# SinOncology/BreakID

Measured on NVIDIA B200. Metric: read_pairs_per_sec_classified_clustered_refined, higher is better.
Workload: dtype u32/i64 integer + f64 (AHC distances)

## Files before the change

### breakid_b200/csrc/bkid_api.cuh

```cuda
#pragma once

#define GRID1(n, t) (unsigned)div_up((long long)(n), (t))

enum CounterSlot {
  CS_G = 0,
  CS_SD_OUT = 16,
  CS_SDF = 20,
  CS_SORT = 28,
  CS_TOTAL = 32,
  CS_HASH_ERR = 40,
  CS_MAXSPAN = 44,
  CS_FATAL = 46,
  CS_ROOTS = 48,
  CS_MISSING = 50,
  CS_DECODE = 52,
  CS_NC = 64,
  CS_XBAD = 65,
  CS_RG_TICKET = 66,
  CS_SORT_HEAP = 67
};

struct Scratch {
  DBuf keys, keys_alt, vals, vals_alt, hist, scan_tmp, a32, b32, c32, d32, e32;
  int ensure(long long n, cudaStream_t st)
// ... 197 lines not shown
  cudaStream_t st = c->st;
  if (n == 0) { CU(c, cudaMemsetAsync(seg_out, 0, (size_t)(nseg + 1) * 4, st)); *n_out = 0; return 0; }
  TRY(c, c->sc.ensure(n, st));
  uint32_t *cnt = c->sc.a32.as<uint32_t>(), *off = c->sc.b32.as<uint32_t>();
  unsigned long long *tot = (unsigned long long *)(c->counters.as<unsigned>() + CS_TOTAL);
  BK_LAUNCH(k4_mask_count, GRID1(n, 256), 256, 0, st, cur, curb, seg, n, X, Y, distance, cnt);
  bk::exclusive_scan<uint32_t, uint32_t>(cnt, off, n, c->sc.scan_tmp.as<unsigned long long>(), tot, st);
  unsigned long long h = 0;
  CU(c, cudaMemcpyAsync(&h, tot, 8, cudaMemcpyDeviceToHost, st));
  CU(c, cudaStreamSynchronize(st));
  BK_LAUNCH(k4_mask_write, GRID1(n, 256), 256, 0, st, cur, curb, n, cnt, off, cur_out, curb_out);
  BK_LAUNCH(k4_new_offsets, GRID1(nseg + 1, 256), 256, 0, st, seg, nseg, off, n, h, seg_out);
  *n_out = (long long)h;
  return 0;
}

static int compact_pass(bkid_ctx *c, const uint32_t *cur, const uint32_t *curb, const uint32_t *seg, long long n, int nseg, const uint32_t *keep,
                        uint32_t *cur_out, uint32_t *curb_out, uint32_t *seg_out, uint32_t *off_keep , long long *n_out)
{
  cudaStream_t st = c->st;
  if (n == 0) { CU(c, cudaMemsetAsync(seg_out, 0, (size_t)(nseg + 1) * 4, st)); *n_out = 0; return 0; }
  unsigned long long *tot = (unsigned long long *)(c->counters.as<unsigned>() + CS_TOTAL);
  bk::exclusive_scan<uint32_t, uint32_t>(keep, off_keep, n, c->sc.scan_tmp.as<unsigned long long>(), tot, st);
  unsigned long long h = 0;
  CU(c, cudaMemcpyAsync(&h, tot, 8, cudaMemcpyDeviceToHost, st));
  CU(c, cudaStreamSynchronize(st));
  BK_LAUNCH(compact_write, GRID1(n, 256), 256, 0, st, cur, curb, keep, off_keep, n, cur_out, curb_out);
  BK_LAUNCH(k4_new_offsets, GRID1(nseg + 1, 256), 256, 0, st, seg, nseg, off_keep, n, h, seg_out);
  *n_out = (long long)h;
  return 0;
}

static int remove_isolated_all(bkid_ctx *c, const uint32_t *cur0, const uint32_t *curb0, const uint32_t *seg0, long long n0, int nseg,
                               const uint32_t *X, const uint32_t *Y, double w)
{
  cudaStream_t st = c->st;
  long long distance = (long long)w;
  size_t m = (size_t)std::max<long long>(n0, 1) * 4 + 64, sb = (size_t)(nseg + 2) * 4;
  TRY(c, c->cur1.ensure(m, 0, st)); TRY(c, c->curb1.ensure(m, 0, st)); TRY(c, c->seg1.ensure(sb, 0, st));
  DBuf &ca = c->sc.c32, &cb = c->sc.d32;
  TRY(c, c->sc.ensure(n0 + 8, st));
  TRY(c, c->tmpG.ensure(3 * sb + m * 2, 0, st));
  uint32_t *segA = c->tmpG.as<uint32_t>(), *segB = segA + (nseg + 2);
  uint32_t *curA = ca.as<uint32_t>(), *curbA = cb.as<uint32_t>();
  uint32_t *work_cur = c->tmpG.as<uint32_t>() + 3 * (nseg + 2);
  uint32_t *work_curb = work_cur + std::max<long long>(n0, 1) + 8;
  if (n0 > 0) {
    CU(c, cudaMemcpyAsync(work_cur, cur0, (size_t)n0 * 4, cudaMemcpyDeviceToDevice, st));
    CU(c, cudaMemcpyAsync(work_curb, curb0, (size_t)n0 * 4, cudaMemcpyDeviceToDevice, st));
  }
  TRY(c, sort_current_by(c, work_cur, n0, X, seg0, nseg));
  long long na = 0, nb2 = 0;
  TRY(c, mask_pass(c, work_cur, work_curb, seg0, n0, nseg, X, Y, distance, curA, curbA, segA, &na));
  TRY(c, sort_current_by(c, curA, na, Y, segA, nseg));
  TRY(c, mask_pass(c, curA, curbA, segA, na, nseg, X, Y, distance, c->cur1.as<uint32_t>(), c->curb1.as<uint32_t>(), segB, &nb2));
  TRY(c, sort_current_by(c, c->cur1.as<uint32_t>(), nb2, X, segB, nseg));
  CU(c, cudaMemcpyAsync(c->seg1.p, segB, (size_t)(nseg + 1) * 4, cudaMemcpyDeviceToDevice, st));
  c->n1 = nb2;
  return 0;
}

static int cluster_ahc(bkid_ctx *c, const uint32_t *cur, const uint32_t *curb, const uint32_t *seg, long long n, int nseg, const uint32_t *X, const uint32_t *Y, double thr_d)
{
  cudaStream_t st = c->st;
  c->n2 = 0;
  c->roots_per_bucket.assign(nseg, 0);
  if (n == 0) return 0;
  long long thr = (long long)thr_d;
  SubTimer T_(st);
  TRY(c, c->sc.ensure(n + 8, st));
  DBuf &LX = c->tmpA, &LY = c->tmpB;
  TRY(c, LX.ensure((size_t)n * 4 + 16, 0, st)); TRY(c, LY.ensure((size_t)n * 4 + 16, 0, st));
  BK_LAUNCH(gather_u32, GRID1(n, 256), 256, 0, st, X, cur, n, LX.as<uint32_t>());
  BK_LAUNCH(gather_u32, GRID1(n, 256), 256, 0, st, Y, cur, n, LY.as<uint32_t>());
  uint64_t *key = c->sc.keys.as<uint64_t>();
  uint32_t *val = c->sc.vals.as<uint32_t>();
  uint32_t *head = c->sc.a32.as<uint32_t>(), *hex = c->sc.b32.as<uint32_t>();
  unsigned long long *stmp = c->sc.scan_tmp.as<unsigned long long>();
  unsigned long long *tot = (unsigned long long *)(c->counters.as<unsigned>() + CS_TOTAL);
  int bbits = 1; while ((1ll << bbits) < nseg + 1) ++bbits;
  BK_LAUNCH(ahc_key_bx, GRID1(n, 256), 256, 0, st, curb, LX.as<uint32_t>(), n, key, val);
  bk::radix_sort_pairs(key, val, n, 0, 32 + bbits, c->sc.rt(), st);
  BK_LAUNCH(ahc_gap_heads, GRID1(n, 256), 256, 0, st, key, n, thr, head);
  bk::exclusive_scan<uint32_t, uint32_t>(head, hex, n, stmp, tot, st);
  unsigned long long npiece = 0;
  CU(c, cudaMemcpyAsync(&npiece, tot, 8, cudaMemcpyDeviceToHost, st)); CU(c, cudaStreamSynchronize(st));
  int pbits = 1; while ((1ull << pbits) < npiece + 1) ++pbits;
  BK_LAUNCH(ahc_key_group, GRID1(n, 256), 256, 0, st, head, hex, val, LY.as<uint32_t>(), n, key);
  bk::radix_sort_pairs(key, val, n, 0, 32 + pbits, c->sc.rt(), st);
  BK_LAUNCH(ahc_gap_heads, GRID1(n, 256), 256, 0, st, key, n, thr, head);
  bk::exclusive_scan<uint32_t, uint32_t>(head, hex, n, stmp, tot, st);
  unsigned long long ncomp64 = 0;
  CU(c, cudaMemcpyAsync(&ncomp64, tot, 8, cudaMemcpyDeviceToHost, st)); CU(c, cudaStreamSynchronize(st));
  uint32_t ncomp = (uint32_t)ncomp64;
  int cbits = 1; while ((1ull << cbits) < ncomp64 + 1) ++cbits;
  BK_LAUNCH(ahc_key_group, GRID1(n, 256), 256, 0, st, head, hex, val, (const uint32_t *)nullptr, n, key);
  bk::radix_sort_pairs(key, val, n, 0, 32 + cbits, c->sc.rt(), st);
  BK_LAUNCH(ahc_comp_heads, GRID1(n, 256), 256, 0, st, key, n, head);
  T_.mark("ahc: component sorts");
  DBuf &T = c->tmpC;
  size_t nc1 = (size_t)ncomp + 2;
  size_t bytes = nc1 * (4 + 4 + 4 + 8 + 8 + 8 + 8 + 4 + 8 + 8 + 4 + 8 + 4 + 4) + (size_t)n * (4 + 4 + 4) + (size_t)(nseg + 2) * (4 + 4 + 4 + 4) + 4096;
  TRY(c, T.ensure(bytes, 0, st));
  CU(c, cudaMemsetAsync(T.p, 0, bytes, st));
  char *bp = (char *)T.p;
  auto take = [&](size_t b) { char *r = bp; bp += (b + 15) & ~(size_t)15; return r; };
  uint32_t *comp_off = (uint32_t *)take(nc1 * 4), *comp_bucket = (uint32_t *)take(nc1 * 4);
  int32_t *hi_oc = (int32_t *)take(nc1 * 4);
  unsigned long long *pts_sz = (unsigned long long *)take(nc1 * 8), *row_sz = (unsigned long long *)take(nc1 * 8);
  unsigned long long *pts_off = (unsigned long long *)take(nc1 * 8), *row_off = (unsigned long long *)take(nc1 * 8);
  uint32_t *comp_nnodes = (uint32_t *)take(nc1 * 4);
  unsigned long long *comp_pts_used = (unsigned long long *)take(nc1 * 8), *comp_row_used = (unsigned long long *)take(nc1 * 8);
  int32_t *comp_head_j = (int32_t *)take(nc1 * 4);
  double *comp_head_d = (double *)take(nc1 * 8);
  int32_t *comp_flag = (int32_t *)take(nc1 * 4);
  uint32_t *comp_cursor = (uint32_t *)take(nc1 * 4);
  uint32_t *comp_of_point = (uint32_t *)take((size_t)n * 4);
  uint32_t *comp_leaf = (uint32_t *)take((size_t)n * 4);
  int32_t *lo_oc = (int32_t *)take((size_t)n * 4);
  uint32_t *bucket_comp_off = (uint32_t *)take((size_t)(nseg + 2) * 4);
  int32_t *bucket_flag = (int32_t *)take((size_t)(nseg + 2) * 4);
  unsigned *merges_pb = (unsigned *)take((size_t)(nseg + 2) * 4);
  uint32_t *bucket_first_root = (uint32_t *)take((size_t)(nseg + 2) * 4);
  BK_LAUNCH(ahc_comp_fill, GRID1(n, 256), 256, 0, st, key, head, val, n, curb, comp_off, comp_bucket, comp_of_point);
  CU(c, cudaMemcpyAsync(comp_leaf, val, (size_t)n * 4, cudaMemcpyDeviceToDevice, st));
  { uint32_t nn = (uint32_t)n; CU(c, cudaMemcpyAsync(comp_off + ncomp, &nn, 4, cudaMemcpyHostToDevice, st)); CU(c, cudaStreamSynchronize(st)); }
  BK_LAUNCH(ahc_comp_static, GRID1(ncomp, 128), 128, 0, st, comp_off, comp_leaf, comp_bucket, comp_of_point, seg, ncomp, lo_oc, hi_oc, pts_sz, row_sz);
  unsigned long long *tot2 = tot + 1;
  bk::exclusive_scan<unsigned long long, unsigned long long>(pts_sz, pts_off, ncomp, stmp, tot, st);
  bk::exclusive_scan<unsigned long long, unsigned long long>(row_sz, row_off, ncomp, stmp, tot2, st);
  unsigned long long pool[2] = {0, 0};
  std::vector<uint32_t> seg_h((size_t)nseg + 1);
  CU(c, cudaMemcpyAsync(seg_h.data(), seg, (size_t)(nseg + 1) * 4, cudaMemcpyDeviceToHost, st));
  CU(c, cudaMemcpyAsync(pool, tot, 16, cudaMemcpyDeviceToHost, st)); CU(c, cudaStreamSynchronize(st));
  bool have_large = false;
  const uint32_t RG_LO = 512u;
  for (int b = 0; b < nseg; ++b) have_large |= seg_h[b + 1] - seg_h[b] >= RG_LO;
  if ((pool[0] * 4 + pool[1] * 12) > (100ull << 30)) return fail(c, BKID_ERR_NOMEM, "AHC component too large for the row pools");
  BK_LAUNCH(ahc_bucket_comp_off, GRID1(nseg + 1, 128), 128, 0, st, comp_bucket, ncomp, (uint32_t)nseg, bucket_comp_off);
  DBuf &NB = c->tmpD;
  size_t nn2 = (size_t)2 * n + 2;
  size_t nbytes = nn2 * (1 + 4 + 8 + 8 + 4 + 4 + 8 + 4 + 4 + 4) + (size_t)n * (8 + 4) + pool[0] * 4 + pool[1] * 12 + 8192;
  TRY(c, NB.ensure(nbytes, 0, st));
  bp = (char *)NB.p;
  AhcView v;
  memset(&v, 0, sizeof v);
  v.seg_off = seg; v.X = LX.as<uint32_t>(); v.Y = LY.as<uint32_t>();
  v.comp_off = comp_off; v.comp_leaf = comp_leaf; v.comp_bucket = comp_bucket; v.lo_oc = lo_oc; v.hi_oc = hi_oc;
  v.pts_off = pts_off; v.row_off = row_off;
  v.node_best_d = (double *)take(nn2 * 8);
  v.node_pts = (unsigned long long *)take(nn2 * 8); v.node_row = (unsigned long long *)take(nn2 * 8);
  v.row_d = (double *)take(pool[1] * 8 + 8);
  v.ev_d = (double *)take((size_t)n * 8 + 8);
  v.node_npts = (uint32_t *)take(nn2 * 4); v.node_rowlen = (uint32_t *)take(nn2 * 4);
  v.node_best_t = (int32_t *)take(nn2 * 4); v.node_grank = (int32_t *)take(nn2 * 4);
  v.node_ma = (int32_t *)take(nn2 * 4); v.node_mb = (int32_t *)take(nn2 * 4);
  v.pts_pool = (uint32_t *)take(pool[0] * 4 + 8); v.row_t = (int32_t *)take(pool[1] * 4 + 8);
  v.ev_first = (int32_t *)take((size_t)n * 4 + 8);
  v.node_root = (uint8_t *)take(nn2);
  v.comp_nnodes = comp_nnodes; v.comp_pts_used = comp_pts_used; v.comp_row_used = comp_row_used;
  v.comp_head_j = comp_head_j; v.comp_head_d = comp_head_d; v.comp_flag = comp_flag; v.comp_cursor = comp_cursor;
  v.thr = (double)thr;
  T_.mark("ahc: tables+alloc");
  BK_LAUNCH(ahc_components, GRID1(ncomp, 4), 128, 0, st, v, ncomp);
  T_.mark("ahc: components kernel");
  BK_LAUNCH(ahc_bucket_flags, GRID1(ncomp, 128), 128, 0, st, comp_flag, comp_bucket, ncomp, bucket_flag);
  T_.mark("ahc: bucket flags");
  if (T_.on) {
    std::vector<int32_t> hf(ncomp); std::vector<uint32_t> hoff(ncomp + 1), hnn(ncomp);
    cudaMemcpyAsync(hf.data(), comp_flag, (size_t)ncomp * 4, cudaMemcpyDeviceToHost, st);
    cudaMemcpyAsync(hoff.data(), comp_off, (size_t)(ncomp + 1) * 4, cudaMemcpyDeviceToHost, st);
    cudaMemcpyAsync(hnn.data(), comp_nnodes, (size_t)ncomp * 4, cudaMemcpyDeviceToHost, st);
    cudaStreamSynchronize(st);
    long nf = 0, maxc = 0, merges = 0, fl_pts = 0;
    for (uint32_t i = 0; i < ncomp; ++i) { uint32_t cs = hoff[i + 1] - hoff[i]; nf += hf[i] != 0; if (hf[i]) fl_pts += cs; maxc = std::max<long>(maxc, cs); merges += hnn[i] - cs; }
    fprintf(stderr, "[bkid-timing] ncomp %u flagged %ld (points %ld) max comp %ld merges %ld points %lld buckets %d\n", ncomp, nf, fl_pts, maxc, merges, n, nseg);
  }
  BK_LAUNCH(ahc_replay_rank, (unsigned)nseg, RK_THREADS, 49 * 512, st, v, bucket_comp_off, (uint32_t)nseg, bucket_flag, 0u, RG_LO);
  T_.mark("ahc: replay rank form");
  BK_LAUNCH(ahc_replay_smem, (unsigned)nseg, 32, 49 * 900, st, v, bucket_comp_off, (uint32_t)nseg, bucket_flag, 0u, 900u);
  BK_LAUNCH(ahc_replay_smem, (unsigned)nseg, 32, 49 * 4096, st, v, bucket_comp_off, (uint32_t)nseg, bucket_flag, 900u, 4096u);
  T_.mark("ahc: replay smem (flagged)");
  if (have_large) {
    DBuf &RG = c->tmpF;
    size_t nn = (size_t)n + 8;
    TRY(c, RG.ensure(nn * (8 + 4 + 4 + 4 + 4 + 4 + 4 + 1) + (size_t)(nseg + 2) * 4 + 256, 0, st));
    char *q = (char *)RG.p;
    RankGlobal g;
    g.pm = (double *)q; q += nn * 8;
    g.slot_comp = (uint32_t *)q; q += nn * 4;
    g.first = (int32_t *)q; q += nn * 4;
    g.rank = (uint32_t *)q; q += nn * 4;
    g.order = (uint32_t *)q; q += nn * 4;
    g.is_head = (uint32_t *)q; q += nn * 4;
    uint32_t *head_excl = (uint32_t *)q; q += nn * 4;
    uint32_t *bucket_events = (uint32_t *)q; q += (size_t)(nseg + 2) * 4;
    g.tie = (uint8_t *)q;
    uint32_t *head_pos = c->sc.e32.as<uint32_t>();
    CU(c, cudaMemsetAsync(bucket_events, 0, (size_t)(nseg + 2) * 4, st));
    CU(c, cudaMemsetAsync(g.is_head, 0, nn * 4, st));
    BK_LAUNCH(ahc_rg_bucket_events, GRID1(ncomp, 128), 128, 0, st, v, ncomp, bucket_events);
    BK_LAUNCH(ahc_rg_prepare, GRID1(ncomp, 128), 128, 0, st, v, g, ncomp, bucket_flag, RG_LO);
    {
      uint64_t *rk = c->sc.keys.as<uint64_t>();
      uint32_t *rv = c->sc.vals.as<uint32_t>();
      BK_LAUNCH(ahc_rg_sortkeys, GRID1(n, 256), 256, 0, st, v, g, curb, n, bucket_flag, RG_LO, rk, rv);
      bk::radix_sort_pairs(rk, rv, n, 0, 64, c->sc.rt(), st);
      BK_LAUNCH(ahc_rg_bucketkeys, GRID1(n, 256), 256, 0, st, curb, rv, n, rk);
      bk::radix_sort_pairs(rk, rv, n, 0, bbits, c->sc.rt(), st);
// ... 1579 lines not shown
```

### breakid_b200/csrc/bkid_cluster.cuh

```cuda
#pragma once

struct AhcView {
  const uint32_t *seg_off;
  const uint32_t *X, *Y;
  const uint32_t *comp_off;
  const uint32_t *comp_leaf;
  const uint32_t *comp_bucket;
  const int32_t *lo_oc;
  const int32_t *hi_oc;
  const unsigned long long *pts_off, *row_off;
  uint8_t *node_root;
  uint32_t *node_npts;
  unsigned long long *node_pts;
  unsigned long long *node_row;
  uint32_t *node_rowlen;
  int32_t *node_best_t;
  double *node_best_d;
  int32_t *node_grank;
  int32_t *node_ma, *node_mb;
  uint32_t *pts_pool;
  int32_t *row_t;
  double *row_d;
  uint32_t *comp_nnodes;
  unsigned long long *comp_pts_used, *comp_row_used;
// ... 568 lines not shown
  uint32_t b = point_bucket[e];
  if (bucket_flag[b] || v.seg_off[b + 1] - v.seg_off[b] < n_lo) return;
  if (!(g.pm[e] < 1.0e300)) return;
  uint32_t comp = g.slot_comp[e], lbase = v.comp_off[comp], c = v.comp_off[comp + 1] - lbase;
  v.node_grank[2 * lbase + c + ((uint32_t)e - lbase)] = (int32_t)g.rank[e];
}

__global__ void __launch_bounds__(32) ahc_bucket_exact(AhcView v, const uint32_t *__restrict__ bucket_comp_off, uint32_t nb, const int32_t *__restrict__ bucket_flag, uint32_t n_lo)
{
  uint32_t b = blockIdx.x;
  if (b >= nb || !bucket_flag[b]) return;
  if (v.seg_off[b + 1] - v.seg_off[b] < n_lo) return;
  const unsigned lane = threadIdx.x & 31;
  uint32_t c0 = bucket_comp_off[b], c1 = bucket_comp_off[b + 1];
  uint32_t nleaf = v.seg_off[b + 1] - v.seg_off[b];
  for (uint32_t comp = c0; comp < c1; ++comp) {
    CompCtx cc = make_cc(v, comp);
    ahc_comp_init(v, cc);
    for (uint32_t j = 1; j < cc.c; ++j) ahc_find_best<true>(v, cc, j);
    ahc_comp_head(v, cc);
  }
  int32_t g = 0;
  while (true) {
    double bd = 1.7976931348623157e308; int32_t bg = -1; uint32_t bc = 0xffffffffu;
    for (uint32_t comp = c0 + lane; comp < c1; comp += 32) {
      int32_t hj = v.comp_head_j[comp];
      if (hj < 0) continue;
      uint32_t lbase = v.comp_off[comp], c = v.comp_off[comp + 1] - lbase;
      double d = v.comp_head_d[comp];
      int32_t gi = (uint32_t)hj < c ? (int32_t)(v.comp_leaf[lbase + hj] - v.seg_off[b]) : (int32_t)nleaf + v.node_grank[2 * lbase + hj];
      if (bg < 0 || d < bd || (d == bd && gi > bg)) { bd = d; bg = gi; bc = comp; }
    }
    for (int o = 16; o; o >>= 1) {
      double od = __shfl_xor_sync(0xffffffffu, bd, o);
      int32_t og = __shfl_xor_sync(0xffffffffu, bg, o);
      uint32_t oc = __shfl_xor_sync(0xffffffffu, bc, o);
      if (og >= 0 && (bg < 0 || od < bd || (od == bd && og > bg))) { bd = od; bg = og; bc = oc; }
    }
    if (bg < 0 || !(bd <= v.thr)) break;
    CompCtx cc = make_cc(v, bc);
    ahc_merge<true>(v, cc, g);
    ++g;
  }
}

__global__ void ahc_key_bx(const uint32_t *__restrict__ bucket_of, const uint32_t *__restrict__ X, long long np, uint64_t *__restrict__ key, uint32_t *__restrict__ val)
{
  long long p = (long long)blockIdx.x * blockDim.x + threadIdx.x;
  if (p < np) { key[p] = ((uint64_t)bucket_of[p] << 32) | X[p]; val[p] = (uint32_t)p; }
}
__global__ void ahc_gap_heads(const uint64_t *__restrict__ key, long long np, long long thr, uint32_t *__restrict__ head)
{
  long long p = (long long)blockIdx.x * blockDim.x + threadIdx.x;
  if (p >= np) return;
  unsigned h = 1;
  if (p > 0 && (key[p] >> 32) == (key[p - 1] >> 32)) {
    long long gap = (long long)(key[p] & 0xffffffffull) - (long long)(key[p - 1] & 0xffffffffull);
    h = gap > thr ? 1u : 0u;
  }
  head[p] = h;
}
__global__ void ahc_key_group(const uint32_t *__restrict__ head, const uint32_t *__restrict__ head_excl, const uint32_t *__restrict__ val,
                              const uint32_t *__restrict__ low, long long np, uint64_t *__restrict__ key)
{
  long long p = (long long)blockIdx.x * blockDim.x + threadIdx.x;
  if (p >= np) return;
  uint32_t g = head_excl[p] - (head[p] ? 0u : 1u);
  key[p] = ((uint64_t)g << 32) | (low ? low[val[p]] : val[p]);
}
__global__ void ahc_comp_heads(const uint64_t *__restrict__ key, long long np, uint32_t *__restrict__ head)
{
  long long p = (long long)blockIdx.x * blockDim.x + threadIdx.x;
  if (p < np) head[p] = (p == 0 || (key[p] >> 32) != (key[p - 1] >> 32)) ? 1u : 0u;
}
__global__ void ahc_comp_fill(const uint64_t *__restrict__ key, const uint32_t *__restrict__ head, const uint32_t *__restrict__ val, long long np,
                              const uint32_t *__restrict__ bucket_of, uint32_t *__restrict__ comp_off, uint32_t *__restrict__ comp_bucket,
                              uint32_t *__restrict__ comp_of_point)
{
  long long p = (long long)blockIdx.x * blockDim.x + threadIdx.x;
  if (p >= np) return;
  uint32_t comp = (uint32_t)(key[p] >> 32);
  comp_of_point[val[p]] = comp;
  if (head[p]) { comp_off[comp] = (uint32_t)p; comp_bucket[comp] = bucket_of[val[p]]; }
}
__global__ void ahc_comp_static(const uint32_t *__restrict__ comp_off, const uint32_t *__restrict__ comp_leaf, const uint32_t *__restrict__ comp_bucket,
                                const uint32_t *__restrict__ comp_of_point, const uint32_t *__restrict__ seg_off, uint32_t ncomp,
                                int32_t *__restrict__ lo_oc, int32_t *__restrict__ hi_oc, unsigned long long *__restrict__ pts_sz, unsigned long long *__restrict__ row_sz)
{
  uint32_t comp = blockIdx.x * blockDim.x + threadIdx.x;
  if (comp >= ncomp) return;
  uint32_t s = comp_off[comp], e = comp_off[comp + 1], c = e - s;
  uint32_t pb = seg_off[comp_bucket[comp]], pe = seg_off[comp_bucket[comp] + 1];
  for (uint32_t q = s; q < e; ++q) {
    int32_t leaf = (int32_t)(comp_leaf[q] - pb);
    if (q > s && comp_leaf[q - 1] + 1 == comp_leaf[q]) lo_oc[q] = lo_oc[q - 1];
    else lo_oc[q] = leaf - 1;
  }
  long long r = (long long)pe - 1;
  while (r >= (long long)pb && comp_of_point[r] == comp) --r;
  hi_oc[comp] = (int32_t)(r - (long long)pb);
  pts_sz[comp] = (unsigned long long)c * (c + 1) / 2 + 1;
  row_sz[comp] = (unsigned long long)c * (c > 0 ? c - 1 : 0) / 2 + 1;
}
__global__ void ahc_bucket_comp_off(const uint32_t *__restrict__ comp_bucket, uint32_t ncomp, uint32_t nb, uint32_t *__restrict__ bucket_comp_off)
{
  uint32_t b = blockIdx.x * blockDim.x + threadIdx.x;
  if (b > nb) return;
  uint32_t lo = 0, hi = ncomp;
  while (lo < hi) { uint32_t m = (lo + hi) / 2; if (comp_bucket[m] < b) lo = m + 1; else hi = m; }
  bucket_comp_off[b] = lo;
}
__global__ void ahc_bucket_flags(const int32_t *__restrict__ comp_flag, const uint32_t *__restrict__ comp_bucket, uint32_t ncomp, int32_t *__restrict__ bucket_flag)
{
  uint32_t comp = blockIdx.x * blockDim.x + threadIdx.x;
  if (comp < ncomp && comp_flag[comp]) bucket_flag[comp_bucket[comp]] = 1;
}

__global__ void ahc_final_roots(AhcView v, uint32_t ncomp, uint64_t *__restrict__ key, uint32_t *__restrict__ val , unsigned *__restrict__ count,
                                unsigned *__restrict__ merges_per_bucket)
{
  uint32_t comp = blockIdx.x * blockDim.x + threadIdx.x;
  if (comp >= ncomp) return;
  uint32_t lbase = v.comp_off[comp], c = v.comp_off[comp + 1] - lbase, nn = v.comp_nnodes[comp];
  if (nn > c) atomicAdd(&merges_per_bucket[v.comp_bucket[comp]], nn - c);
  for (uint32_t j = c; j < nn; ++j)
    if (v.node_root[2 * lbase + j]) {
      unsigned o = atomicAdd(count, 1u);
      key[o] = ((uint64_t)v.comp_bucket[comp] << 32) | (uint32_t)v.node_grank[2 * lbase + j];
      val[o] = 2 * lbase + j;
    }
}
__global__ void ahc_root_sizes(AhcView v, const uint64_t *__restrict__ key, const uint32_t *__restrict__ node, uint32_t nroot, uint32_t *__restrict__ size,
                               uint32_t *__restrict__ head)
{
  uint32_t r = blockIdx.x * blockDim.x + threadIdx.x;
  if (r >= nroot) return;
  size[r] = v.node_npts[node[r]];
  head[r] = (r == 0 || (key[r] >> 32) != (key[r - 1] >> 32)) ? 1u : 0u;
}
__global__ void ahc_root_firsts(const uint32_t *__restrict__ head, uint32_t nroot, const uint64_t *__restrict__ key, uint32_t *__restrict__ bucket_first_root)
{
  uint32_t r = blockIdx.x * blockDim.x + threadIdx.x;
  if (r < nroot && head[r]) bucket_first_root[(uint32_t)(key[r] >> 32)] = r;
}
__global__ void __launch_bounds__(128) ahc_emit(AhcView v, const uint64_t *__restrict__ key, const uint32_t *__restrict__ node, const uint32_t *__restrict__ out_off,
                                                const uint32_t *__restrict__ bucket_first_root, uint32_t nroot,
                                                uint32_t *__restrict__ out_point, int32_t *__restrict__ out_cluster, uint32_t *__restrict__ out_bucket)
{
  uint32_t r = blockIdx.x * (blockDim.x >> 5) + (threadIdx.x >> 5);
  if (r >= nroot) return;
  const unsigned lane = threadIdx.x & 31;
  uint32_t b = (uint32_t)(key[r] >> 32);
  uint32_t nd = node[r], n = v.node_npts[nd], o = out_off[r];
  unsigned long long po = v.node_pts[nd];
  uint32_t pbase = v.seg_off[b];
  int32_t k = (int32_t)(r - bucket_first_root[b]);
  for (uint32_t i = lane; i < n; i += 32) {
    out_point[o + i] = pbase + v.pts_pool[po + i];
    out_cluster[o + i] = k;
    out_bucket[o + i] = b;
  }
}

__global__ void fast_sweep(const uint32_t *__restrict__ cur, const uint32_t *__restrict__ seg_off, uint32_t nb, const uint32_t *__restrict__ coord,
                           double w, int min_reads, uint32_t *__restrict__ kout , uint32_t *__restrict__ keep )
{
// ... 105 lines not shown
```

### breakid_b200/csrc/prims.cuh

```cuda
#pragma once
#include <atomic>
#include <cuda_runtime.h>
#include <stdint.h>

#define BK_CUDA(x)                                                          \
  do {                                                                      \
    cudaError_t e__ = (x);                                                  \
    if (e__ != cudaSuccess) { bk_set_cuda_error(e__, __FILE__, __LINE__); return BKID_ERR_CUDA; } \
  } while (0)

void bk_set_cuda_error(cudaError_t e, const char *file, int line);
extern thread_local long long g_bk_launches;
extern bool g_bk_prof_on;
void bk_prof_begin(const char *name, cudaStream_t st);
void bk_prof_end(cudaStream_t st);
#define BK_LAUNCH(kernel, grid, block, smem, stream, ...)                   \
  do {                                                                      \
    if (g_bk_prof_on) bk_prof_begin(#kernel, (stream));                     \
    kernel<<<(grid), (block), (smem), (stream)>>>(__VA_ARGS__);            \
    if (g_bk_prof_on) bk_prof_end((stream));                                \
    ++g_bk_launches;                                                        \
  } while (0)

namespace bk {

static inline int div_up(long long a, long long b) { return (int)((a + b - 1) / b); }

__device__ __forceinline__ unsigned lane_id() { return threadIdx.x & 31; }

template <typename T>
__device__ __forceinline__ T warp_incl_scan(T v)
{
#pragma unroll
  for (int o = 1; o < 32; o <<= 1) {
    T u = __shfl_up_sync(0xffffffffu, v, o);
    if (lane_id() >= (unsigned)o) v += u;
  }
  return v;
}

template <typename T>
__device__ __forceinline__ T warp_sum(T v)
{
#pragma unroll
  for (int o = 16; o; o >>= 1) v += __shfl_xor_sync(0xffffffffu, v, o);
  return v;
}

template <typename T>
__device__ __forceinline__ T block_excl_scan(T v, T *sh, T &total)
{
  unsigned w = threadIdx.x >> 5, l = lane_id(), nw = blockDim.x >> 5;
  T inc = warp_incl_scan(v);
  if (l == 31) sh[w] = inc;
  __syncthreads();
  if (w == 0) {
    T s = l < nw ? sh[l] : T(0);
    T si = warp_incl_scan(s);
    sh[l] = si - s;
    if (l == 31) sh[32] = si;
  }
  __syncthreads();
  T r = inc - v + sh[w];
  total = sh[32];
  __syncthreads();
  return r;
}

constexpr int SCAN_THREADS = 512;
constexpr int SCAN_ITEMS = 8;
constexpr int SCAN_TILE = SCAN_THREADS * SCAN_ITEMS;

template <typename InT>
__global__ void __launch_bounds__(SCAN_THREADS) scan_tile_sums(const InT *__restrict__ in, long long n, unsigned long long *__restrict__ tile_sum)
{
  __shared__ unsigned long long sh[33];
  long long base = (long long)blockIdx.x * SCAN_TILE;
  unsigned long long s = 0;
#pragma unroll
  for (int k = 0; k < SCAN_ITEMS; ++k) {
    long long i = base + (long long)k * SCAN_THREADS + threadIdx.x;
    if (i < n) s += (unsigned long long)in[i];
  }
  unsigned long long tot;
  block_excl_scan<unsigned long long>(s, sh, tot);
  if (threadIdx.x == 0) tile_sum[blockIdx.x] = tot;
}

__global__ void __launch_bounds__(1024) scan_tile_offsets(unsigned long long *__restrict__ tile_sum, int ntiles, unsigned long long *__restrict__ total_out)
{
  __shared__ unsigned long long sh[33];
  unsigned long long carry = 0;
  for (int b = 0; b < ntiles; b += 1024) {
    int i = b + threadIdx.x;
    unsigned long long v = i < ntiles ? tile_sum[i] : 0ull, tot;
    unsigned long long ex = block_excl_scan<unsigned long long>(v, sh, tot);
    if (i < ntiles) tile_sum[i] = carry + ex;
    carry += tot;
  }
  if (threadIdx.x == 0 && total_out) *total_out = carry;
}

template <typename InT, typename OutT>
__global__ void __launch_bounds__(SCAN_THREADS) scan_tiles(const InT *in, long long n, const unsigned long long *__restrict__ tile_off, OutT *out)
{
  __shared__ unsigned long long sh[33];
  long long base = (long long)blockIdx.x * SCAN_TILE + (long long)threadIdx.x * SCAN_ITEMS;
  unsigned long long v[SCAN_ITEMS], s = 0;
#pragma unroll
  for (int k = 0; k < SCAN_ITEMS; ++k) { long long i = base + k; v[k] = i < n ? (unsigned long long)in[i] : 0ull; s += v[k]; }
  unsigned long long tot;
  unsigned long long ex = block_excl_scan<unsigned long long>(s, sh, tot) + tile_off[blockIdx.x];
#pragma unroll
  for (int k = 0; k < SCAN_ITEMS; ++k) { long long i = base + k; if (i < n) out[i] = (OutT)ex; ex += v[k]; }
}

template <typename InT, typename OutT>
static inline void exclusive_scan(const InT *in, OutT *out, long long n, unsigned long long *tmp, unsigned long long *total_out, cudaStream_t st)
{
  if (n <= 0) { if (total_out) cudaMemsetAsync(total_out, 0, 8, st); return; }
  int ntiles = div_up(n, SCAN_TILE);
  BK_LAUNCH((scan_tile_sums<InT>), ntiles, SCAN_THREADS, 0, st, in, n, tmp);
  BK_LAUNCH(scan_tile_offsets, 1, 1024, 0, st, tmp, ntiles, total_out);
  BK_LAUNCH((scan_tiles<InT, OutT>), ntiles, SCAN_THREADS, 0, st, in, n, tmp, out);
}
static inline size_t scan_tmp_elems(long long n) { return (size_t)div_up(n > 0 ? n : 1, SCAN_TILE) + 1; }

constexpr int OS_THREADS = 256;
constexpr int OS_WARPS = OS_THREADS / 32;
constexpr int OS_ITEMS = 16;
constexpr int OS_TILE = OS_THREADS * OS_ITEMS;
constexpr int OS_MAX_PASSES = 8;
constexpr unsigned OS_FLAG_AGG = 1u << 30, OS_FLAG_PREFIX = 2u << 30, OS_VAL_MASK = (1u << 30) - 1u;
constexpr size_t OS_SMEM = (size_t)OS_TILE * 12 + (size_t)OS_WARPS * 256 * 4 + 2 * 256 * 4 + 40 * 4;

__global__ void __launch_bounds__(256) os_hist(const uint64_t *__restrict__ keys, const uint32_t *__restrict__ n_dev, uint32_t n_host, int lo_bit, int npass,
                                               uint32_t *__restrict__ ghist )
{
  __shared__ uint32_t h[OS_MAX_PASSES][256];
  for (int p = 0; p < npass; ++p) h[p][threadIdx.x] = 0;
  __syncthreads();
  const uint32_t n = n_dev ? *n_dev : n_host;
  for (uint32_t i = blockIdx.x * 256u + threadIdx.x; i < n; i += gridDim.x * 256u) {
    uint64_t k = keys[i] >> lo_bit;
    for (int p = 0; p < npass; ++p) { atomicAdd(&h[p][(uint32_t)k & 255u], 1u); k >>= 8; }
  }
  __syncthreads();
  for (int p = 0; p < npass; ++p) { uint32_t v = h[p][threadIdx.x]; if (v) atomicAdd(&ghist[p * 256 + threadIdx.x], v); }
}

__global__ void __launch_bounds__(256) os_hist_scan(uint32_t *__restrict__ ghist, int npass)
{
  __shared__ uint32_t sh[33];
  for (int p = 0; p < npass; ++p) {
    uint32_t v = ghist[p * 256 + threadIdx.x], tot;
    uint32_t ex = block_excl_scan<uint32_t>(v, sh, tot);
    ghist[p * 256 + threadIdx.x] = ex;
  }
}

__global__ void __launch_bounds__(OS_THREADS) os_pass(const uint64_t *__restrict__ kin, const uint32_t *__restrict__ vin, uint64_t *__restrict__ kout, uint32_t *__restrict__ vout,
                                                      const uint32_t *__restrict__ n_dev, uint32_t n_host, int shift, const uint32_t *__restrict__ ghist_excl,
                                                      uint32_t *__restrict__ status , uint32_t *__restrict__ ticket)
{
  extern __shared__ __align__(16) unsigned char os_smem[];
  uint64_t *skey = reinterpret_cast<uint64_t *>(os_smem);
  uint32_t *sval = reinterpret_cast<uint32_t *>(os_smem + (size_t)OS_TILE * 8);
  uint32_t *whist = sval + OS_TILE;
  uint32_t *toff = whist + OS_WARPS * 256;
  uint32_t *gbase = toff + 256;
  uint32_t *misc = gbase + 256;
  if (threadIdx.x == 0) misc[0] = atomicAdd(ticket, 1u);
  for (int i = threadIdx.x; i < OS_WARPS * 256; i += OS_THREADS) whist[i] = 0;
  __syncthreads();
  const uint32_t tile = misc[0];
  const uint32_t n = n_dev ? *n_dev : n_host;
  const uint32_t base = tile * (uint32_t)OS_TILE;
  if (base >= n) return;
  const uint32_t cnt = min((uint32_t)OS_TILE, n - base);
  const unsigned w = threadIdx.x >> 5, l = threadIdx.x & 31, ltmask = (1u << l) - 1u;
  uint64_t k[OS_ITEMS];
  uint32_t v[OS_ITEMS];
  uint16_t rk[OS_ITEMS];
#pragma unroll
  for (int r = 0; r < OS_ITEMS; ++r) {
    uint32_t i = w * (32u * OS_ITEMS) + (uint32_t)r * 32u + l;
    bool ok = i < cnt;
    k[r] = ok ? kin[base + i] : ~0ull;
    v[r] = ok ? vin[base + i] : 0u;
  }
  uint32_t *wh = whist + w * 256;
#pragma unroll
  for (int r = 0; r < OS_ITEMS; ++r) {
    uint32_t i = w * (32u * OS_ITEMS) + (uint32_t)r * 32u + l;
    bool ok = i < cnt;
    unsigned d = ok ? (unsigned)(k[r] >> shift) & 255u : 256u;
    unsigned m = __match_any_sync(0xffffffffu, d);
    int leader = __ffs(m) - 1;
    uint32_t old = 0;
    if ((int)l == leader && ok) { old = wh[d]; wh[d] = old + __popc(m); }
    old = __shfl_sync(0xffffffffu, old, leader);
    rk[r] = (uint16_t)(old + __popc(m & ltmask));
    __syncwarp();
  }
  __syncthreads();
  uint32_t c = 0;
  {
    const unsigned d = threadIdx.x;
#pragma unroll
    for (int ww = 0; ww < OS_WARPS; ++ww) { uint32_t t = whist[ww * 256 + d]; whist[ww * 256 + d] = c; c += t; }
    volatile uint32_t *st = status + (size_t)tile * 256 + d;
    if (tile == 0) *st = OS_FLAG_PREFIX | c;
    else {
      *st = OS_FLAG_AGG | c;
      uint32_t excl = 0;
      for (int t = (int)tile - 1; t >= 0; --t) {
        volatile uint32_t *q = status + (size_t)t * 256 + d;
        uint32_t sv;
        do { sv = *q; } while ((sv >> 30) == 0u);
        excl += sv & OS_VAL_MASK;
        if ((sv >> 30) == 2u) break;
      }
      *st = OS_FLAG_PREFIX | (excl + c);
      gbase[d] = ghist_excl[d] + excl;
    }
    if (tile == 0) gbase[d] = ghist_excl[d];
    uint32_t tot;
    toff[d] = block_excl_scan<uint32_t>(c, misc + 1, tot);
  }
  __syncthreads();
#pragma unroll
  for (int r = 0; r < OS_ITEMS; ++r) {
    uint32_t i = w * (32u * OS_ITEMS) + (uint32_t)r * 32u + l;
    if (i < cnt) {
      unsigned d = (unsigned)(k[r] >> shift) & 255u;
      uint32_t pos = toff[d] + wh[d] + rk[r];
      skey[pos] = k[r]; sval[pos] = v[r];
    }
  }
  __syncthreads();
  for (uint32_t i = threadIdx.x; i < cnt; i += OS_THREADS) {
    uint64_t kk = skey[i];
    unsigned d = (unsigned)(kk >> shift) & 255u;
    uint32_t dst = gbase[d] + (i - toff[d]);
    kout[dst] = kk; vout[dst] = sval[i];
  }
}

struct RadixTmp {
  uint64_t *keys_alt; uint32_t *vals_alt; uint32_t *hist; unsigned long long *scan_tmp;
};
static inline size_t radix_hist_elems(long long n)
{
  size_t tiles = (size_t)div_up(n > 0 ? n : 1, OS_TILE);
  return (size_t)OS_MAX_PASSES * 256 + 64 + (size_t)OS_MAX_PASSES * tiles * 256;
}

static inline int radix_sort_pairs(uint64_t *keys, uint32_t *vals, long long n, int lo_bit, int hi_bit, const RadixTmp &t, cudaStream_t st, const uint32_t *n_dev = nullptr)
{
  if (n <= 1 || hi_bit <= lo_bit) return 0;
  if (n >= (1ll << 30)) return -1;
  static std::atomic<unsigned long long> attr_done{0};
  int dev = 0; cudaGetDevice(&dev);
  if (!((attr_done.load(std::memory_order_acquire) >> (dev & 63)) & 1)) {
    cudaFuncSetAttribute(os_pass, cudaFuncAttributeMaxDynamicSharedMemorySize, (int)OS_SMEM);
    attr_done.fetch_or(1ull << (dev & 63), std::memory_order_release);
  }
  int npass = (hi_bit - lo_bit + 7) / 8;
  if (npass > OS_MAX_PASSES) npass = OS_MAX_PASSES;
  int ntiles = div_up(n, OS_TILE);
  uint32_t *ghist = t.hist, *tickets = t.hist + OS_MAX_PASSES * 256, *status = t.hist + OS_MAX_PASSES * 256 + 64;
  cudaMemsetAsync(t.hist, 0, ((size_t)OS_MAX_PASSES * 256 + 64 + (size_t)npass * ntiles * 256) * 4, st);
  int hgrid = ntiles < 148 * 8 ? ntiles : 148 * 8;
  BK_LAUNCH(os_hist, hgrid, 256, 0, st, keys, n_dev, (uint32_t)n, lo_bit, npass, ghist);
  BK_LAUNCH(os_hist_scan, 1, 256, 0, st, ghist, npass);
  uint64_t *ki = keys, *ko = t.keys_alt;
  uint32_t *vi = vals, *vo = t.vals_alt;
  for (int p = 0; p < npass; ++p) {
    BK_LAUNCH(os_pass, ntiles, OS_THREADS, OS_SMEM, st, ki, vi, ko, vo, n_dev, (uint32_t)n, lo_bit + 8 * p, ghist + p * 256, status + (size_t)p * ntiles * 256, tickets + p);
    uint64_t *tk = ki; ki = ko; ko = tk;
    uint32_t *tv = vi; vi = vo; vo = tv;
  }
  if (npass & 1) {
    cudaMemcpyAsync(keys, ki, (size_t)n * 8, cudaMemcpyDeviceToDevice, st);
    cudaMemcpyAsync(vals, vi, (size_t)n * 4, cudaMemcpyDeviceToDevice, st);
  }
  return npass;
}

}
```

Baseline: 52.66 billion.

## Add single-cluster small radix sort and small scan, drop host syncs in AHC

Adds a single-block exclusive scan and a thread-block-cluster radix sort that keeps all passes in distributed shared memory. Inputs up to about 64K elements use these instead of the multi-kernel paths, and an env var can turn them off. It also removes two host round-trips in AHC: the piece count readback is replaced by a bit width bounded by n, and the comp_off sentinel is now written by ahc_comp_fill. The aim is to cut launch and sync latency on small inputs, at the cost of more sort passes because pbits is now derived from n.

```diff
diff --git a/breakid_b200/csrc/bkid_api.cuh b/breakid_b200/csrc/bkid_api.cuh
--- a/breakid_b200/csrc/bkid_api.cuh
+++ b/breakid_b200/csrc/bkid_api.cuh
@@ -303,10 +303,8 @@
   BK_LAUNCH(ahc_key_bx, GRID1(n, 256), 256, 0, st, curb, LX.as<uint32_t>(), n, key, val);
   bk::radix_sort_pairs(key, val, n, 0, 32 + bbits, c->sc.rt(), st);
   BK_LAUNCH(ahc_gap_heads, GRID1(n, 256), 256, 0, st, key, n, thr, head);
-  bk::exclusive_scan<uint32_t, uint32_t>(head, hex, n, stmp, tot, st);
-  unsigned long long npiece = 0;
-  CU(c, cudaMemcpyAsync(&npiece, tot, 8, cudaMemcpyDeviceToHost, st)); CU(c, cudaStreamSynchronize(st));
-  int pbits = 1; while ((1ull << pbits) < npiece + 1) ++pbits;
+  bk::exclusive_scan<uint32_t, uint32_t>(head, hex, n, stmp, nullptr, st);
+  int pbits = 1; while ((1ll << pbits) < n + 1) ++pbits;
   BK_LAUNCH(ahc_key_group, GRID1(n, 256), 256, 0, st, head, hex, val, LY.as<uint32_t>(), n, key);
   bk::radix_sort_pairs(key, val, n, 0, 32 + pbits, c->sc.rt(), st);
   BK_LAUNCH(ahc_gap_heads, GRID1(n, 256), 256, 0, st, key, n, thr, head);
@@ -345,7 +343,6 @@
   uint32_t *bucket_first_root = (uint32_t *)take((size_t)(nseg + 2) * 4);
   BK_LAUNCH(ahc_comp_fill, GRID1(n, 256), 256, 0, st, key, head, val, n, curb, comp_off, comp_bucket, comp_of_point);
   CU(c, cudaMemcpyAsync(comp_leaf, val, (size_t)n * 4, cudaMemcpyDeviceToDevice, st));
-  { uint32_t nn = (uint32_t)n; CU(c, cudaMemcpyAsync(comp_off + ncomp, &nn, 4, cudaMemcpyHostToDevice, st)); CU(c, cudaStreamSynchronize(st)); }
   BK_LAUNCH(ahc_comp_static, GRID1(ncomp, 128), 128, 0, st, comp_off, comp_leaf, comp_bucket, comp_of_point, seg, ncomp, lo_oc, hi_oc, pts_sz, row_sz);
   unsigned long long *tot2 = tot + 1;
   bk::exclusive_scan<unsigned long long, unsigned long long>(pts_sz, pts_off, ncomp, stmp, tot, st);
diff --git a/breakid_b200/csrc/bkid_cluster.cuh b/breakid_b200/csrc/bkid_cluster.cuh
--- a/breakid_b200/csrc/bkid_cluster.cuh
+++ b/breakid_b200/csrc/bkid_cluster.cuh
@@ -674,6 +674,7 @@
   uint32_t comp = (uint32_t)(key[p] >> 32);
   comp_of_point[val[p]] = comp;
   if (head[p]) { comp_off[comp] = (uint32_t)p; comp_bucket[comp] = bucket_of[val[p]]; }
+  if (p == np - 1) comp_off[comp + 1] = (uint32_t)np;
 }
 __global__ void ahc_comp_static(const uint32_t *__restrict__ comp_off, const uint32_t *__restrict__ comp_leaf, const uint32_t *__restrict__ comp_bucket,
                                 const uint32_t *__restrict__ comp_of_point, const uint32_t *__restrict__ seg_off, uint32_t ncomp,
diff --git a/breakid_b200/csrc/prims.cuh b/breakid_b200/csrc/prims.cuh
--- a/breakid_b200/csrc/prims.cuh
+++ b/breakid_b200/csrc/prims.cuh
@@ -1,7 +1,9 @@
 #pragma once
 #include <atomic>
+#include <cooperative_groups.h>
 #include <cuda_runtime.h>
 #include <stdint.h>
+#include <stdlib.h>
 
 #define BK_CUDA(x)                                                          \
   do {                                                                      \
@@ -115,10 +117,43 @@
   for (int k = 0; k < SCAN_ITEMS; ++k) { long long i = base + k; if (i < n) out[i] = (OutT)ex; ex += v[k]; }
 }
 
+constexpr int SMALL_SCAN_THREADS = 1024;
+constexpr int SMALL_SCAN_ITEMS = 8;
+constexpr int SMALL_SCAN_CHUNK = SMALL_SCAN_THREADS * SMALL_SCAN_ITEMS;
+constexpr long long SMALL_SCAN_MAX = 8ll * SMALL_SCAN_CHUNK;
+
+template <typename InT, typename OutT>
+__global__ void __launch_bounds__(SMALL_SCAN_THREADS) small_scan(const InT *in, long long n, OutT *out, unsigned long long *__restrict__ total_out)
+{
+  __shared__ unsigned long long sh[33];
+  unsigned long long carry = 0;
+  for (long long b = 0; b < n; b += SMALL_SCAN_CHUNK) {
+    long long base = b + (long long)threadIdx.x * SMALL_SCAN_ITEMS;
+    unsigned long long v[SMALL_SCAN_ITEMS], s = 0, tot;
+#pragma unroll
+    for (int k = 0; k < SMALL_SCAN_ITEMS; ++k) { long long i = base + k; v[k] = i < n ? (unsigned long long)in[i] : 0ull; s += v[k]; }
+    unsigned long long ex = block_excl_scan<unsigned long long>(s, sh, tot) + carry;
+#pragma unroll
+    for (int k = 0; k < SMALL_SCAN_ITEMS; ++k) { long long i = base + k; if (i < n) out[i] = (OutT)ex; ex += v[k]; }
+    carry += tot;
+  }
+  if (threadIdx.x == 0 && total_out) *total_out = carry;
+}
+
+static inline bool small_prims_on()
+{
+  const char *e = getenv("BKID_SMALL_PRIMS");
+  return !(e && e[0] == '0' && e[1] == 0);
+}
+
 template <typename InT, typename OutT>
 static inline void exclusive_scan(const InT *in, OutT *out, long long n, unsigned long long *tmp, unsigned long long *total_out, cudaStream_t st)
 {
   if (n <= 0) { if (total_out) cudaMemsetAsync(total_out, 0, 8, st); return; }
+  if (n <= SMALL_SCAN_MAX && small_prims_on()) {
+    BK_LAUNCH((small_scan<InT, OutT>), 1, SMALL_SCAN_THREADS, 0, st, in, n, out, total_out);
+    return;
+  }
   int ntiles = div_up(n, SCAN_TILE);
   BK_LAUNCH((scan_tile_sums<InT>), ntiles, SCAN_THREADS, 0, st, in, n, tmp);
   BK_LAUNCH(scan_tile_offsets, 1, 1024, 0, st, tmp, ntiles, total_out);
@@ -247,6 +282,106 @@
   }
 }
 
+constexpr int SS_THREADS = 512;
+constexpr int SS_WARPS = SS_THREADS / 32;
+constexpr int SS_ITEMS = 16;
+constexpr int SS_CTA_MAX = SS_THREADS * SS_ITEMS;
+constexpr int SS_CLUSTER = 8;
+constexpr long long SMALL_SORT_MAX = (long long)SS_CLUSTER * SS_CTA_MAX;
+static inline size_t ss_smem(int T) { return (size_t)T * 24 + ((size_t)SS_WARPS * 256 + 2 * 256 + 40) * 4; }
+
+__global__ void __launch_bounds__(SS_THREADS, 1) small_sort(uint64_t *__restrict__ keys, uint32_t *__restrict__ vals, const uint32_t *__restrict__ n_dev, uint32_t n_host,
+                                                            int lo_bit, int npass, int T)
+{
+  namespace cg = cooperative_groups;
+  cg::cluster_group cl = cg::this_cluster();
+  extern __shared__ __align__(16) unsigned char ss_smem_raw[];
+  uint64_t *skey = reinterpret_cast<uint64_t *>(ss_smem_raw);
+  uint32_t *sval = reinterpret_cast<uint32_t *>(ss_smem_raw + (size_t)T * 16);
+  uint32_t *whist = sval + 2 * T;
+  uint32_t *dcnt = whist + SS_WARPS * 256;
+  uint32_t *gbase = dcnt + 256;
+  uint32_t *scr = gbase + 256;
+  const unsigned rank = cl.block_rank(), nrank = cl.num_blocks();
+  const uint32_t n = n_dev ? min(*n_dev, n_host) : n_host;
+  const uint32_t base = rank * (uint32_t)T;
+  const uint32_t cnt = base < n ? min((uint32_t)T, n - base) : 0u;
+  const int R = T / (32 * SS_WARPS);
+  const unsigned w = threadIdx.x >> 5, l = threadIdx.x & 31, ltmask = (1u << l) - 1u;
+  uint32_t *wh = whist + w * 256;
+  uint64_t k[SS_ITEMS];
+  uint32_t v[SS_ITEMS];
+  uint32_t rk[SS_ITEMS];
+  for (int p = 0; p < npass; ++p) {
+    const int shift = lo_bit + 8 * p;
+    const uint64_t *ksrc = p == 0 ? keys + base : skey + (size_t)(p & 1) * T;
+    const uint32_t *vsrc = p == 0 ? vals + base : sval + (size_t)(p & 1) * T;
+#pragma unroll
+    for (int r = 0; r < SS_ITEMS; ++r) {
+      uint32_t i = w * (32u * R) + (uint32_t)r * 32u + l;
+      bool ok = r < R && i < cnt;
+      k[r] = ok ? ksrc[i] : 0ull;
+      v[r] = ok ? vsrc[i] : 0u;
+    }
+    for (int i = threadIdx.x; i < SS_WARPS * 256; i += SS_THREADS) whist[i] = 0;
+    __syncthreads();
+#pragma unroll
+    for (int r = 0; r < SS_ITEMS; ++r) {
+      if (r < R) {
+        uint32_t i = w * (32u * R) + (uint32_t)r * 32u + l;
+        bool ok = i < cnt;
+        unsigned d = ok ? (unsigned)(k[r] >> shift) & 255u : 256u;
+        unsigned m = __match_any_sync(0xffffffffu, d);
+        int leader = __ffs(m) - 1;
+        uint32_t old = 0;
+        if ((int)l == leader && ok) { old = wh[d]; wh[d] = old + __popc(m); }
+        old = __shfl_sync(0xffffffffu, old, leader);
+        rk[r] = old + __popc(m & ltmask);
+        __syncwarp();
+      }
+    }
+    __syncthreads();
+    if (threadIdx.x < 256) {
+      const unsigned d = threadIdx.x;
+      uint32_t c = 0;
+#pragma unroll
+      for (int ww = 0; ww < SS_WARPS; ++ww) { uint32_t t = whist[ww * 256 + d]; whist[ww * 256 + d] = c; c += t; }
+      dcnt[d] = c;
+    }
+    cl.sync();
+    uint32_t tot_d = 0, below = 0;
+    if (threadIdx.x < 256) {
+      for (unsigned q = 0; q < nrank; ++q) {
+        uint32_t x = cl.map_shared_rank(dcnt, q)[threadIdx.x];
+        tot_d += x;
+        if (q < rank) below += x;
+      }
+    }
+    uint32_t tot;
+    uint32_t ex = block_excl_scan<uint32_t>(tot_d, scr, tot);
+    if (threadIdx.x < 256) gbase[threadIdx.x] = ex + below;
+    __syncthreads();
+    const bool last = p == npass - 1;
+    uint64_t *dk = skey + (size_t)((p + 1) & 1) * T;
+    uint32_t *dv = sval + (size_t)((p + 1) & 1) * T;
+#pragma unroll
+    for (int r = 0; r < SS_ITEMS; ++r) {
+      uint32_t i = w * (32u * R) + (uint32_t)r * 32u + l;
+      if (r < R && i < cnt) {
+        unsigned d = (unsigned)(k[r] >> shift) & 255u;
+        uint32_t pos = gbase[d] + wh[d] + rk[r];
+        if (last) { keys[pos] = k[r]; vals[pos] = v[r]; }
+        else {
+          unsigned q = pos / (uint32_t)T, o = pos - q * (uint32_t)T;
+          cl.map_shared_rank(dk, q)[o] = k[r];
+          cl.map_shared_rank(dv, q)[o] = v[r];
+        }
+      }
+    }
+    cl.sync();
+  }
+}
+
 struct RadixTmp {
   uint64_t *keys_alt; uint32_t *vals_alt; uint32_t *hist; unsigned long long *scan_tmp;
 };
@@ -264,10 +399,25 @@
   int dev = 0; cudaGetDevice(&dev);
   if (!((attr_done.load(std::memory_order_acquire) >> (dev & 63)) & 1)) {
     cudaFuncSetAttribute(os_pass, cudaFuncAttributeMaxDynamicSharedMemorySize, (int)OS_SMEM);
+    cudaFuncSetAttribute(small_sort, cudaFuncAttributeMaxDynamicSharedMemorySize, (int)ss_smem(SS_CTA_MAX));
     attr_done.fetch_or(1ull << (dev & 63), std::memory_order_release);
   }
   int npass = (hi_bit - lo_bit + 7) / 8;
   if (npass > OS_MAX_PASSES) npass = OS_MAX_PASSES;
+  if (n <= SMALL_SORT_MAX && small_prims_on()) {
+    const int T = div_up(div_up(n, SS_CLUSTER), SS_THREADS) * SS_THREADS, nb = div_up(n, T);
+    cudaLaunchConfig_t cfg = {};
+    cudaLaunchAttribute at[1];
+    at[0].id = cudaLaunchAttributeClusterDimension;
+    at[0].val.clusterDim.x = (unsigned)nb; at[0].val.clusterDim.y = 1; at[0].val.clusterDim.z = 1;
+    cfg.gridDim = dim3((unsigned)nb); cfg.blockDim = dim3(SS_THREADS); cfg.dynamicSmemBytes = ss_smem(T); cfg.stream = st;
+    cfg.attrs = at; cfg.numAttrs = 1;
+    if (g_bk_prof_on) bk_prof_begin("small_sort", st);
+    cudaLaunchKernelEx(&cfg, small_sort, keys, vals, n_dev, (uint32_t)n, lo_bit, npass, T);
+    if (g_bk_prof_on) bk_prof_end(st);
+    ++g_bk_launches;
+    return npass;
+  }
   int ntiles = div_up(n, OS_TILE);
   uint32_t *ghist = t.hist, *tickets = t.hist + OS_MAX_PASSES * 256, *status = t.hist + OS_MAX_PASSES * 256 + 64;
   cudaMemsetAsync(t.hist, 0, ((size_t)OS_MAX_PASSES * 256 + 64 + (size_t)npass * ntiles * 256) * 4, st);
```

Result: faster. 54.33 billion, median of 6 (+3.2%).
